# 4l3x4ndre/Metadata-Augmented-UNET-for-LST-NDVI

Measured on AMD Instinct MI355X. Metric: train images/sec (256x256x6->2 U-Net, B=32/GPU), higher is better.
Workload: dtype bf16; 1 GPU; metadata-unet base_filters=64, 32x6x256x256 tiles + 4-dim metadata per GPU, fwd+MSE+bwd+AdamW (src/train.py:243-256); global_batch=32, parallelism=dp1, sync_bn=False, launch=hipGraph replay of the captured step

## Files before the change

### include/mau_hip.h

```cpp
#ifndef MAU_HIP_H
#define MAU_HIP_H

#include <stddef.h>
#include <stdint.h>

#ifdef __cplusplus
extern "C" {
#endif

#define MAU_F32 0
#define MAU_BF16 1
#define MAU_F16 2

#define MAU_OK 0
#define MAU_ERR_ARG 1
#define MAU_ERR_HIP 2
#define MAU_ERR_DEVICE 3

typedef void* mau_stream_t;

#define MAU_ABI_VERSION 5
int mau_abi_version(void);
const char* mau_last_error(void);
int mau_device_check(void);

int mau_nchw_to_nhwc(const float* src, void* dst, int dtype, int N, int C, int H, int W, int ld,
                     mau_stream_t stream);
int mau_nhwc_to_nchw(const void* src, float* dst, int dtype, int N, int C, int H, int W, int ld,
                     mau_stream_t stream);

int mau_pack_tile_onehot(const unsigned char* cls_a, const unsigned char* cls_b, const float* cont,
                         const unsigned char* flip, void* out, int ldo, int dtype, int N, int H, int W,
                         int num_classes, int ncont, mau_stream_t stream);
int mau_flip_rows(const float* src, float* dst, const unsigned char* flip, int N, int C, int H, int W,
                  mau_stream_t stream);

int mau_conv3x3_kc(int dtype);
size_t mau_conv3x3_packed_elems(int dtype, int nout, int nin);
int mau_conv3x3_pack_weights(const float* w_oihw, void* wf, void* wd, int dtype, int Cout, int Cin,
                             mau_stream_t stream);
size_t mau_conv3x3_pack_desc_bytes(void);
int mau_conv3x3_pack_desc_fill(void* descs_host, int index, const float* w_oihw, void* wf, void* wd, int dtype, int Cout,
                               int Cin, int tile0, int* next_tile_host);
int mau_conv3x3_pack_weights_multi(const void* descs, int n, int total_tiles, int dtype, mau_stream_t stream);
int mau_conv3x3_num_pixel_tiles(int dtype, int N, int H, int W, int Cout);
int mau_conv3x3_fwd_pool(const void* x, int ldx, int C0, const void* wpk, const float* bias, const float* post_scale,
                         const float* post_shift, void* y, int ldy, int Cout, void* pooled, int ldpool, int dtype, int N, int H,
                         int W, mau_stream_t stream);
int mau_conv3x3_variant(int dtype, int N, int H, int W, int Cin, int Cout, int* tile_rows_host, int* waves_host, int* cout_block_host,
                        int* k_groups_host);
int mau_conv3x3_first_max_channels(void);
int mau_conv3x3_first_rows(int N, int H, int W);
size_t mau_conv3x3_first_wgrad_ws_elems(int N, int H, int W, int Cout);
int mau_conv3x3_first_wgrad(const void* x8, const void* dz, int lddz, float* dw_oihw, float* ws, int Cin, int Cout, int dtype, int N,
                            int H, int W, mau_stream_t stream);
int mau_conv3x3_first_fwd(const float* x_nchw, int Cin, const float* w_oihw, const float* bias, const float* post_scale,
                          const float* post_shift, void* y, int ldy, int Cout, float* slab, void* x8, int dtype, int N, int H,
                          int W, mau_stream_t stream);
int mau_conv3x3_fwd(const void* x, int ldx, int C0, const float* emb, void* emb_ws, int E, const void* wpk,
                    const float* bias, const float* post_scale, const float* post_shift, void* y, int ldy,
                    int Cout, float* slab, int dtype, int N, int H, int W, mau_stream_t stream);
int mau_conv3x3_fwd2(const void* x, int ldx, int C0, const void* x1, int ldx1, int C1, const float* emb, void* emb_ws,
                     int E, const void* wpk, const float* bias, const float* post_scale, const float* post_shift,
                     void* y, int ldy, int Cout, float* slab, int dtype, int N, int H, int W, mau_stream_t stream);
int mau_conv3x3_wgrad_splits(int dtype, int N, int H, int W, int Cout, int Cin);
size_t mau_conv3x3_wgrad_acc_elems(int dtype, int N, int H, int W, int Cout, int Cin);
int mau_conv3x3_wgrad(const void* x, int ldx, int C0, const float* emb, void* emb_ws, int E, const void* dy,
                      int lddy, int Cout, float* acc, int dtype, int N, int H, int W, mau_stream_t stream);
int mau_conv3x3_wgrad2(const void* x, int ldx, int C0, const void* x1, int ldx1, int C1, const float* emb, void* emb_ws,
                       int E, const void* dy, int lddy, int Cout, float* acc, int dtype, int N, int H, int W,
                       mau_stream_t stream);
int mau_conv3x3_unpack_wgrad(const float* acc, int nsplit, float* dw_oihw, int Cout, int Cin,
                             mau_stream_t stream);

size_t mau_reduce_rows_ws_elems(int rows, int M);
int mau_reduce_tickets_elems(void);
int mau_reduce_rows_f64(const float* slab, int rows, int M, int ldrow, double* sums, double* ws, unsigned* tickets,
                        mau_stream_t stream);
int mau_reduce_rows_f64_f32(const float* slab, int rows, int M, int ldrow, double* sums, float* sums32,
                            double* ws, unsigned* tickets, double append, mau_stream_t stream);
int mau_reduce_rows_f32(const float* slab, int rows, int M, int ldrow, float* out, double* ws, unsigned* tickets,
                        mau_stream_t stream);
int mau_bn_stats_sums_f64(const float* slab, int rows, int C, double* sums, double* ws, unsigned* tickets, double append,
                          mau_stream_t stream);
int mau_bn_finalize_train(const double* sums, double count, const float* gamma, const float* beta,
                          float* running_mean, float* running_var, int64_t* num_batches_tracked,
                          float momentum, float eps, float* scale, float* shift, float* mean,
                          float* invstd, int C, mau_stream_t stream);
size_t mau_bn_stats_ws_elems(int rows, int C);
int mau_bn_stats_finalize_train(const float* slab, int rows, double count, const float* gamma, const float* beta,
                                float* running_mean, float* running_var, int64_t* num_batches_tracked,
                                float momentum, float eps, float* scale, float* shift, float* mean, float* invstd,
                                double* ws, unsigned* tickets, int C, mau_stream_t stream);
int mau_bn_coeffs_eval(const float* gamma, const float* beta, const float* running_mean,
                       const float* running_var, float eps, float* scale, float* shift, float* mean,
                       float* invstd, int C, mau_stream_t stream);
int mau_bn_relu_apply(const void* y, int ldy, const float* scale, const float* shift, void* a, int lda,
                      int dtype, int64_t npix, int C, mau_stream_t stream);
int mau_bn_relu_apply_pool(const void* y, int ldy, const float* scale, const float* shift, void* a, int lda,
                           void* pooled, int ldp, unsigned short* argidx, int dtype, int N, int H, int W, int C,
                           mau_stream_t stream);
int mau_bn_relu_bwd_reduce(const void* da, int ldda, const void* y, int ldy, const float* scale,
                           const float* shift, const float* mean, const float* invstd, float* slab,
                           int ldslab, int dtype, int64_t npix, int C, mau_stream_t stream);
int mau_bn_relu_bwd_apply(const void* da, int ldda, const void* y, int ldy, const float* scale,
                          const float* shift, const float* mean, const float* invstd, const double* sums,
                          double count, void* dy, int lddy, int dtype, int64_t npix, int C,
                          mau_stream_t stream);
// ... 127 lines not shown
```

### metadata-augmented-unet-for-lst-ndvi_amd/_lib.py

```python
from __future__ import annotations

import ctypes as C
import os

import torch

_HERE = os.path.dirname(os.path.abspath(__file__))
LIB_PATH = os.environ.get("MAU_LIB") or os.path.join(_HERE, "libmau_hip.so")

MAU_F32 = 0
MAU_BF16 = 1
MAU_F16 = 2
MAU_OPT_ADAMW, MAU_OPT_ADAM, MAU_OPT_SGD = 0, 1, 2

_p, _i, _i64, _f, _d, _sz = C.c_void_p, C.c_int, C.c_int64, C.c_float, C.c_double, C.c_size_t

PROTOTYPES = {
    "mau_abi_version": (_i, []),
    "mau_last_error": (C.c_char_p, []),
    "mau_device_check": (_i, []),
    "mau_nchw_to_nhwc": (_i, [_p, _p, _i, _i, _i, _i, _i, _i, _p]),
    "mau_pack_tile_onehot": (_i, [_p, _p, _p, _p, _p, _i, _i, _i, _i, _i, _i, _i, _p]),
    "mau_flip_rows": (_i, [_p, _p, _p, _i, _i, _i, _i, _p]),
    "mau_nhwc_to_nchw": (_i, [_p, _p, _i, _i, _i, _i, _i, _i, _p]),
    "mau_conv3x3_kc": (_i, [_i]),
    "mau_conv3x3_packed_elems": (_sz, [_i, _i, _i]),
    "mau_conv3x3_pack_weights": (_i, [_p, _p, _p, _i, _i, _i, _p]),
    "mau_conv3x3_pack_desc_bytes": (_sz, []),
    "mau_conv3x3_pack_desc_fill": (_i, [_p, _i, _p, _p, _p, _i, _i, _i, _i, _p]),
    "mau_conv3x3_pack_weights_multi": (_i, [_p, _i, _i, _i, _p]),
    "mau_conv3x3_num_pixel_tiles": (_i, [_i, _i, _i, _i, _i]),
    "mau_conv3x3_variant": (_i, [_i, _i, _i, _i, _i, _i, _p, _p, _p, _p]),
    "mau_conv3x3_first_max_channels": (_i, []),
    "mau_conv3x3_first_rows": (_i, [_i, _i, _i]),
    "mau_conv3x3_first_wgrad_ws_elems": (_sz, [_i, _i, _i, _i]),
    "mau_conv3x3_first_wgrad": (_i, [_p, _p, _i, _p, _p, _i, _i, _i, _i, _i, _i, _p]),
    "mau_conv3x3_first_fwd": (_i, [_p, _i, _p, _p, _p, _p, _p, _i, _i, _p, _p, _i, _i, _i, _i, _p]),
    "mau_conv3x3_fwd": (_i, [_p, _i, _i, _p, _p, _i, _p, _p, _p, _p, _p, _i, _i, _p, _i, _i, _i, _i, _p]),
    "mau_conv3x3_fwd_pool": (_i, [_p, _i, _i, _p, _p, _p, _p, _p, _i, _i, _p, _i, _i, _i, _i, _i, _p]),
    "mau_conv3x3_fwd2": (_i, [_p, _i, _i, _p, _i, _i, _p, _p, _i, _p, _p, _p, _p, _p, _i, _i, _p, _i, _i, _i, _i, _p]),
    "mau_conv3x3_wgrad_splits": (_i, [_i, _i, _i, _i, _i, _i]),
    "mau_conv3x3_wgrad_acc_elems": (_sz, [_i, _i, _i, _i, _i, _i]),
    "mau_conv3x3_wgrad": (_i, [_p, _i, _i, _p, _p, _i, _p, _i, _i, _p, _i, _i, _i, _i, _p]),
    "mau_conv3x3_wgrad2": (_i, [_p, _i, _i, _p, _i, _i, _p, _p, _i, _p, _i, _i, _p, _i, _i, _i, _i, _p]),
    "mau_conv3x3_unpack_wgrad": (_i, [_p, _i, _p, _i, _i, _p]),
    "mau_reduce_rows_ws_elems": (_sz, [_i, _i]),
    "mau_reduce_tickets_elems": (_i, []),
    "mau_reduce_rows_f64": (_i, [_p, _i, _i, _i, _p, _p, _p, _p]),
    "mau_reduce_rows_f64_f32": (_i, [_p, _i, _i, _i, _p, _p, _p, _p, _d, _p]),
    "mau_reduce_rows_f32": (_i, [_p, _i, _i, _i, _p, _p, _p, _p]),
    "mau_bn_stats_sums_f64": (_i, [_p, _i, _i, _p, _p, _p, _d, _p]),
    "mau_bn_finalize_train": (_i, [_p, _d, _p, _p, _p, _p, _p, _f, _f, _p, _p, _p, _p, _i, _p]),
    "mau_bn_stats_ws_elems": (_sz, [_i, _i]),
    "mau_bn_stats_finalize_train": (_i, [_p, _i, _d, _p, _p, _p, _p, _p, _f, _f, _p, _p, _p, _p, _p, _p, _i, _p]),
    "mau_bn_coeffs_eval": (_i, [_p, _p, _p, _p, _f, _p, _p, _p, _p, _i, _p]),
    "mau_bn_relu_apply": (_i, [_p, _i, _p, _p, _p, _i, _i, _i64, _i, _p]),
    "mau_bn_relu_apply_pool": (_i, [_p, _i, _p, _p, _p, _i, _p, _i, _p, _i, _i, _i, _i, _i, _p]),
    "mau_bn_relu_bwd_reduce": (_i, [_p, _i, _p, _i, _p, _p, _p, _p, _p, _i, _i, _i64, _i, _p]),
    "mau_bn_relu_bwd_apply": (_i, [_p, _i, _p, _i, _p, _p, _p, _p, _p, _d, _p, _i, _i, _i64, _i, _p]),
    "mau_bn_bwd_rows": (_i, [_i64]),
    "mau_pool_bn_bwd_reduce": (_i, [_p, _i, _p, _i, _p, _p, _i, _p, _p, _p, _p, _p, _i, _i, _i, _i, _i, _i, _p]),
    "mau_pool_bn_bwd_apply": (_i, [_p, _i, _p, _i, _p, _p, _i, _p, _p, _p, _p, _p, _d, _p, _i, _i, _i, _i, _i, _i, _p]),
    "mau_head_bn_max_channels": (_i, []),
    "mau_head_bn_fwd": (_i, [_p, _i, _p, _p, _p, _p, _p, _i, _i, _i, _i, _i, _i, _p]),
    "mau_head_bn_bwd_reduce": (_i, [_p, _i, _p, _p, _p, _p, _p, _p, _p, _p, _i, _p, _i, _i, _i, _i, _i, _i, _p]),
    "mau_head_bn_bwd_apply": (_i, [_p, _i, _p, _p, _p, _p, _p, _d, _p, _p, _p, _p, _i, _i, _i, _i, _i, _i, _i, _p]),
    "mau_resize_bilinear_bn_fwd": (_i, [_p, _i, _i, _i, _p, _p, _p, _i, _i, _i, _i, _i, _i, _i, _p]),
    "mau_maxpool2x2_fwd": (_i, [_p, _i, _p, _i, _i, _i, _i, _i, _i, _p]),
    "mau_maxpool2x2_bwd": (_i, [_p, _i, _p, _i, _p, _i, _i, _i, _i, _i, _i, _p]),
    "mau_maxpool2x2_bwd_add": (_i, [_p, _i, _p, _i, _p, _i, _p, _i, _i, _i, _i, _i, _i, _p]),
    "mau_resize_bilinear_fwd": (_i, [_p, _i, _i, _i, _p, _i, _i, _i, _i, _i, _i, _i, _p]),
    "mau_resize_bilinear_bwd": (_i, [_p, _i, _i, _i, _i, _p, _i, _i, _i, _i, _i, _i, _p]),
    "mau_copy_channels": (_i, [_p, _i, _p, _i, _i, _i, _i, _i64, _i, _p]),
    "mau_bcast_fill": (_i, [_p, _p, _i, _i, _i, _i, _i, _i, _i, _p]),
    "mau_bcast_bwd_ws_elems": (_sz, [_i, _i, _i]),
    "mau_bcast_bwd": (_i, [_p, _i, _i, _p, _p, _i, _i, _i, _i, _p]),
    "mau_head_fwd": (_i, [_p, _i, _p, _p, _p, _i, _i, _i, _i, _i, _i, _p]),
    "mau_head_mean_ws_elems": (_sz, [_i, _i, _i]),
    "mau_head_mean": (_i, [_p, _i, _p, _p, _p, _p, _p, _p, _p, _i, _i, _i, _i, _i, _i, _p]),
    "mau_head_bwd": (_i, [_p, _i, _p, _p, _p, _p, _i, _p, _i, _i, _i, _i, _i, _i, _p]),
    "mau_head_bwd_rows": (_i, [_i, _i]),
    "mau_head_bwd_rowlen": (_i, [_i, _i]),
    "mau_meta_mlp_fwd": (_i, [_p, _p, _p, _p, _p, _p, _p, _i, _i, _i, _i, _p]),
    "mau_meta_mlp_bwd": (_i, [_p, _p, _p, _p, _p, _p, _p, _p, _p, _p, _i, _i, _i, _i, _p]),
    "mau_lstm_max_hidden": (_i, []),
    "mau_lstm_fwd": (_i, [_p, _p, _p, _p, _p, _p, _p, _p, _i, _i, _i, _p]),
    "mau_lstm_bwd_ws_elems": (_sz, [_i, _i, _i]),
    "mau_lstm_bwd": (_i, [_p, _p, _p, _p, _p, _p, _p, _p, _p, _p, _i, _i, _i, _p]),
    "mau_linear_fwd": (_i, [_p, _p, _p, _p, _i, _i, _i, _p]),
# ... 67 lines not shown
```

### metadata-augmented-unet-for-lst-ndvi_amd/csrc/conv3x3_first.hip

```cpp
#include "igemm_bf16_util.h"

namespace mau {
namespace first {
using namespace igemm;

constexpr int TH = 16, TW = 64, HR = TH + 2, HC = TW + 2, HPIX = HR * HC;
constexpr int NT = 256, NWAVE = NT / 64;
constexpr int LOADS = (HPIX + NT - 1) / NT;
typedef float f32x4v __attribute__((ext_vector_type(4)));

struct P {
  const float* x;
  int Cin;
  const float* w;
  const float* bias;
  const float* post_scale;
  const float* post_shift;
  void* y;
  int ldy, Cout, CoutPad;
  float* slab;
  void* x8;
  int N, H, W, tilesX, tilesY, nTiles;
};

// ... 264 lines not shown

int mau_conv3x3_first_rows(int N, int H, int W) {
  if (N <= 0 || H <= 0 || W <= 0) return 0;
  return mau::first::grid_x(N * mau::ceil_div(H, mau::first::TH) * mau::ceil_div(W, mau::first::TW));
}

int mau_conv3x3_first_fwd(const float* x, int Cin, const float* w, const float* bias, const float* post_scale, const float* post_shift, void* y,
                          int ldy, int Cout, float* slab, void* x8, int dtype, int N, int H, int W, mau_stream_t stream) {
  using namespace mau;
  MAU_REQUIRE(x && w && y && N > 0 && H > 0 && W > 0 && Cout > 0, "conv3x3_first_fwd: bad arguments");
  MAU_REQUIRE(Cin >= 1 && Cin <= 8, "conv3x3_first_fwd: %d input channels (this kernel serves <= 8; use mau_conv3x3_fwd)", Cin);
  MAU_REQUIRE(dtype == MAU_BF16 || dtype == MAU_F16, "conv3x3_first_fwd: 16-bit activation types only (fp32 = parity mode: mau_conv3x3_fwd)");
  MAU_REQUIRE(ldy % 8 == 0 && ldy >= Cout, "conv3x3_first_fwd: ldy must be a multiple of 8 and >= Cout");
  MAU_REQUIRE((post_scale == nullptr) == (post_shift == nullptr), "conv3x3_first_fwd: post_scale and post_shift come together");
  MAU_REQUIRE(!(post_scale != nullptr && slab != nullptr), "conv3x3_first_fwd: post_scale/post_shift and the statistics slab are mutually exclusive");
  MAU_REQUIRE((long long)N * H * W * ldy * 2 < (1ll << 40), "conv3x3_first_fwd: tensor too large");
  first::P p;
  p.x = x;
  p.Cin = Cin;
  p.w = w;
  p.bias = bias;
  p.post_scale = post_scale;
  p.post_shift = post_shift;
  p.y = y;
  p.ldy = ldy;
  p.Cout = Cout;
  p.CoutPad = round_up(Cout, 64);
  p.slab = slab;
  p.x8 = x8;
  p.N = N;
  p.H = H;
  p.W = W;
  p.tilesX = ceil_div(W, first::TW);
  p.tilesY = ceil_div(H, first::TH);
  p.nTiles = N * p.tilesX * p.tilesY;
  return dtype == MAU_F16 ? first::launch<true>(p, (hipStream_t)stream) : first::launch<false>(p, (hipStream_t)stream);
}

}

namespace mau {
namespace firstw {
using namespace igemm;
typedef float f32x4v __attribute__((ext_vector_type(4)));
typedef unsigned u32x2 __attribute__((ext_vector_type(2)));

constexpr int TWW = 32;
constexpr int DZ_BYTES = TWW * 128;
constexpr int XROW = 1024;
constexpr int BUF = DZ_BYTES + 3 * XROW;
constexpr int NT = 256, NWAVE = 4, NDMA = 7;
constexpr int NBT = 6, NCOL = 16 * NBT;

struct WP {
  const void* x8;
  const void* dz;
  int lddz, Cout;
  float* ws;
  int N, H, W, tilesX, nTiles;
};

template <bool F16>
__device__ __forceinline__ void mfma(const u32x4& a, const u32x4& b, f32x4v& c) {
  if constexpr (F16) asm volatile("v_mfma_f32_16x16x32_f16 %0, %1, %2, %0" : "+v"(c) : "v"(a), "v"(b));
  else asm volatile("v_mfma_f32_16x16x32_bf16 %0, %1, %2, %0" : "+v"(c) : "v"(a), "v"(b));
}
template <int OFF_HI>
__device__ __forceinline__ u32x4 tr_frag(unsigned addr_lo, unsigned addr_hi) {
  u32x2 lo, hi;
  asm volatile("ds_read_b64_tr_b16 %0, %2\n\tds_read_b64_tr_b16 %1, %3 offset:%4" : "=&v"(lo), "=&v"(hi) : "v"(addr_lo), "v"(addr_hi), "n"(OFF_HI));
  return __builtin_shufflevector(lo, hi, 0, 1, 2, 3);
}

template <bool F16>
__global__ __launch_bounds__(NT, 2) void first_wgrad_kernel(WP p) {
  extern __shared__ __attribute__((aligned(16))) unsigned char smem[];
  const int tid = threadIdx.x, lane = tid & 63;
  const int wave = __builtin_amdgcn_readfirstlane(tid >> 6);
  const int co0 = blockIdx.y * 64;
  const unsigned lds0 = (unsigned)(size_t)((__attribute__((address_space(3))) unsigned char*)smem) + wave * (2 * BUF);
  const unsigned long long dz_a = (unsigned long long)p.dz, x_a = (unsigned long long)p.x8, zero_a = (unsigned long long)g_zero_page;

  const int dz_px = lane >> 3, dz_ch = lane & 7;
  const bool dz_ch_ok = co0 + 8 * dz_ch < p.lddz;
  auto issue = [&](int tile, int buf) {
    const int txi = tile % p.tilesX, rowi = tile / p.tilesX;
    const int x0 = txi * TWW, y = rowi % p.H;
    unsigned char* dst = smem + wave * (2 * BUF) + buf * BUF;
#pragma unroll
    for (int d = 0; d < 4; ++d) {
      const int gx = x0 + 8 * d + dz_px;
      unsigned long long src = dz_a + 2ull * ((unsigned long long)((long long)rowi * p.W + gx) * (unsigned)p.lddz + (unsigned)(co0 + 8 * dz_ch));
      asm volatile("" : "+v"(src));
      src = (gx < p.W && dz_ch_ok) ? src : zero_a;
      __builtin_amdgcn_global_load_lds((glb_ptr)src, (lds_ptr)(dst + d * 1024), 16, 0, 0);
    }
#pragma unroll
    for (int dy = 0; dy < 3; ++dy) {
      const int gy = y + dy - 1, gx = x0 + lane - 1;
      const bool in = lane < TWW + 2 && gy >= 0 && gy < p.H && gx >= 0 && gx < p.W;
      unsigned long long src = x_a + 16ull * (unsigned long long)((long long)(rowi + dy - 1) * p.W + gx);
      asm volatile("" : "+v"(src));
      src = in ? src : zero_a;
      __builtin_amdgcn_global_load_lds((glb_ptr)src, (lds_ptr)(dst + DZ_BYTES + dy * XROW), 16, 0, 0);
    }
  };
  const int g = lane >> 4, q = (lane >> 2) & 3, pq = lane & 3;
  const unsigned a_lane = (unsigned)((8 * g + q) * 128 + 8 * pq);
  unsigned b_lane[NBT];
#pragma unroll
  for (int j = 0; j < NBT; ++j) b_lane[j] = (unsigned)(DZ_BYTES + (j >> 1) * XROW + (8 * g + q + 2 * (j & 1)) * 16 + 8 * pq);
  f32x4v acc[4][NBT];
#pragma unroll
  for (int t = 0; t < 4; ++t)
#pragma unroll
    for (int j = 0; j < NBT; ++j) acc[t][j] = f32x4v{0.f, 0.f, 0.f, 0.f};

  const int nw = gridDim.x * NWAVE, w0 = blockIdx.x * NWAVE + wave;
  int buf = 0;
  if (w0 < p.nTiles) issue(w0, 0);
  for (int tile = w0; tile < p.nTiles; tile += nw) {
    const bool more = tile + nw < p.nTiles;
    if (more) {
      issue(tile + nw, buf ^ 1);
      wait_vmcnt<NDMA>();
    } else {
      wait_vmcnt<0>();
    }
    const unsigned base = lds0 + buf * BUF;
    u32x4 A[4], B[NBT];
#pragma unroll
    for (int t = 0; t < 4; ++t) A[t] = tr_frag<4 * 128>(base + a_lane + 32 * t, base + a_lane + 32 * t);
#pragma unroll
    for (int j = 0; j < NBT; ++j) B[j] = tr_frag<4 * 16>(base + b_lane[j], base + b_lane[j]);
    asm volatile("s_waitcnt lgkmcnt(0)" ::: "memory");
#pragma unroll
    for (int t = 0; t < 4; ++t)
#pragma unroll
      for (int j = 0; j < NBT; ++j) mfma<F16>(A[t], B[j], acc[t][j]);
    buf ^= 1;
  }
  wait_vmcnt<0>();
  __syncthreads();
  float* red = reinterpret_cast<float*>(smem);
  const int dn = lane & 15, dq = lane >> 4;
  for (int wv = 0; wv < NWAVE; ++wv) {
    if (wave == wv) {
#pragma unroll
      for (int t = 0; t < 4; ++t)
#pragma unroll
        for (int j = 0; j < NBT; ++j)
#pragma unroll
          for (int r = 0; r < 4; ++r) {
            float* e = red + (16 * t + 4 * dq + r) * NCOL + 16 * j + dn;
            *e = wv == 0 ? acc[t][j][r] : *e + acc[t][j][r];
          }
    }
    __syncthreads();
  }
  float* out = p.ws + ((size_t)blockIdx.x * gridDim.y + blockIdx.y) * 64 * NCOL;
  for (int i = tid; i < 64 * NCOL; i += NT) out[i] = red[i];
}

constexpr int SUM_SL = 8, SUM_EL = 32;
__global__ __launch_bounds__(SUM_SL * SUM_EL) void first_wgrad_sum_kernel(const float* __restrict__ ws, int nwg, int coTiles, float* __restrict__ dw, int Cout, int Cin) {
  __shared__ float part[SUM_SL][SUM_EL];
  const int el = threadIdx.x % SUM_EL, sl = threadIdx.x / SUM_EL;
  const int i = blockIdx.x * SUM_EL + el, total = Cout * Cin * 9;
  const int ic = i < total ? i : 0;
  const int tap = ic % 9, ci = (ic / 9) % Cin, co = ic / (9 * Cin);
  const int dy = tap / 3, dx = tap - 3 * dy;
  const int col = 16 * (2 * dy + (dx == 2)) + 8 * (dx == 1) + ci;
  const float* src = ws + (size_t)co * NCOL + col;
  const size_t stride = (size_t)coTiles * 64 * NCOL;
  float s = 0.f;
  int wgi = sl;
  for (; wgi + 7 * SUM_SL < nwg; wgi += 8 * SUM_SL) {
    float v[8];
#pragma unroll
    for (int u = 0; u < 8; ++u) v[u] = src[(size_t)(wgi + u * SUM_SL) * stride];
#pragma unroll
    for (int u = 0; u < 8; ++u) s += v[u];
  }
  for (; wgi < nwg; wgi += SUM_SL) s += src[(size_t)wgi * stride];
  part[sl][el] = s;
  __syncthreads();
  if (sl == 0 && i < total) {
    float o = part[0][el];
#pragma unroll
    for (int k = 1; k < SUM_SL; ++k) o += part[k][el];
    dw[i] = o;
  }
}

static int grid_x(int nTiles) {
  const int cap = device_shape().cus * 2;
  const int need = ceil_div(nTiles, NWAVE);
  return need < cap ? need : cap;
}
}
}

extern "C" {

size_t mau_conv3x3_first_wgrad_ws_elems(int N, int H, int W, int Cout) {
  if (N <= 0 || H <= 0 || W <= 0 || Cout <= 0) return 0;
  return (size_t)mau::firstw::grid_x(N * H * mau::ceil_div(W, mau::firstw::TWW)) * mau::round_up(Cout, 64) * mau::firstw::NCOL;
}

int mau_conv3x3_first_wgrad(const void* x8, const void* dz, int lddz, float* dw, float* ws, int Cin, int Cout, int dtype, int N, int H, int W,
                            mau_stream_t stream) {
  using namespace mau;
  MAU_REQUIRE(x8 && dz && dw && ws && N > 0 && H > 0 && W > 0 && Cout > 0, "conv3x3_first_wgrad: bad arguments");
  MAU_REQUIRE(Cin >= 1 && Cin <= 8, "conv3x3_first_wgrad: %d input channels (this kernel serves <= 8; use mau_conv3x3_wgrad2)", Cin);
  MAU_REQUIRE(dtype == MAU_BF16 || dtype == MAU_F16, "conv3x3_first_wgrad: 16-bit activation types only");
  MAU_REQUIRE(lddz % 8 == 0 && lddz >= Cout && ((uintptr_t)x8 % 16) == 0 && ((uintptr_t)dz % 16) == 0, "conv3x3_first_wgrad: bad lddz / alignment");
  firstw::WP p;
  p.x8 = x8;
  p.dz = dz;
  p.lddz = lddz;
  p.Cout = Cout;
  p.ws = ws;
  p.N = N;
  p.H = H;
  p.W = W;
  p.tilesX = ceil_div(W, firstw::TWW);
  p.nTiles = N * H * p.tilesX;
  const int coTiles = round_up(Cout, 64) / 64;
  const dim3 grid(firstw::grid_x(p.nTiles), coTiles);
  constexpr size_t lds = (size_t)firstw::NWAVE * 2 * firstw::BUF;
  static_assert(lds >= 64 * firstw::NCOL * sizeof(float), "the cross-wave sum fits the DMA buffers");
  hipStream_t st = (hipStream_t)stream;
  if (dtype == MAU_F16) {
    MAU_LDS_ATTR(lds, &firstw::first_wgrad_kernel<true>);
    MAU_LAUNCH(firstw::first_wgrad_kernel<true>, grid, dim3(firstw::NT), lds, st, p);
  } else {
    MAU_LDS_ATTR(lds, &firstw::first_wgrad_kernel<false>);
    MAU_LAUNCH(firstw::first_wgrad_kernel<false>, grid, dim3(firstw::NT), lds, st, p);
  }
  const int rc = check_launch("first_wgrad_kernel");
  if (rc != MAU_OK) return rc;
  MAU_LAUNCH(firstw::first_wgrad_sum_kernel, dim3(ceil_div(Cout * Cin * 9, firstw::SUM_EL)), dim3(firstw::SUM_SL * firstw::SUM_EL), 0, st, ws, (int)grid.x,
             coTiles, dw, Cout, Cin);
  return check_launch("first_wgrad_sum_kernel");
}

}
```

### metadata-augmented-unet-for-lst-ndvi_amd/functional.py

```python
from __future__ import annotations

import contextlib
import dataclasses

import os
from dataclasses import dataclass
from typing import List, Optional, Sequence, Tuple

import torch

from . import _lib
from ._lib import MAU_BF16, MAU_F16, MAU_F32, call, lib

BN_EPS = 1e-5
BN_MOMENTUM = 0.1


def pad8(c: int) -> int:
    return (c + 7) // 8 * 8


def dtype_code(dt: torch.dtype) -> int:
    if dt == torch.float32:
        return MAU_F32
# ... 194 lines not shown
    @staticmethod
    def backward(ctx, g):
        g = _as_nhwc(g)
        N, H, W, _ = g.shape
        out = torch.empty((N, ctx.C, H, W), dtype=torch.float32, device=g.device)
        call("mau_nhwc_to_nchw", g.data_ptr(), out.data_ptr(), dtype_code(g.dtype), N, ctx.C, H, W, _ld(g), _stream())
        return out, None


def to_nchw(a: Act) -> torch.Tensor:
    t = _as_nhwc(a.t.detach())
    N, H, W, _ = t.shape
    out = torch.empty((N, a.C, H, W), dtype=torch.float32, device=t.device)
    call("mau_nhwc_to_nchw", t.data_ptr(), out.data_ptr(), dtype_code(t.dtype), N, a.C, H, W, _ld(t), _stream())
    return out


@dataclass
class BNState:
    training: bool
    C0: int
    momentum: float = BN_MOMENTUM
    eps: float = BN_EPS
    group: object = None
    comm: object = None
    world: int = 1
    grad_enabled: bool = True
    frozen: object = None
    C1: int = 0
    pool: bool = False
    out_view: object = None
    head: object = None
    up_to: object = None
    first: bool = False
    dtype: object = None
    dgrad_first: bool = False


def _all_reduce_(t: torch.Tensor, st: BNState):
    if st.comm is not None:
        st.comm.all_reduce(t, 0, _stream())
    elif st.group is not None:
        from .dist import all_reduce_sum
        all_reduce_sum(t, st.group)


_OVERLAP_WGRAD = int(os.environ.get("MAU_OVERLAP_WGRAD", "2") or 0)
_FUSED_REDUCE = True
_FUSED_BN = True
_FUSED_UP = True
_PACK_MULTI = True
_INFER_POOL_FUSED = True
_FIRST_WGRAD = True
_SIDE_STREAMS = {}


def _side_stream(dev) -> "torch.cuda.Stream":
    s = _SIDE_STREAMS.get(dev)
    if s is None:
        s = _SIDE_STREAMS[dev] = torch.cuda.Stream(device=dev)
    return s


def _join_side_when_backward_ends(dev):
    def join():
        torch.cuda.current_stream(dev).wait_stream(_side_stream(dev))

    torch.autograd.Variable._execution_engine.queue_callback(join)


_DGRAD_FIRST = None


def _conv_fwd(x, x1, st, emb, emb_ws, E, wpk, bias, post, y, Cout, slab, code, N, H, W, stream):
    scale, shift = post if post is not None else (None, None)
    call("mau_conv3x3_fwd2", x.data_ptr(), _ld(x), st.C0, x1.data_ptr() if x1 is not None else None,
         _ld(x1) if x1 is not None else 0, st.C1 if x1 is not None else 0, emb.data_ptr() if E else None,
         emb_ws.data_ptr() if E else None, E, wpk.data_ptr(), bias.data_ptr() if bias is not None else None,
         scale.data_ptr() if scale is not None else None, shift.data_ptr() if shift is not None else None,
         y.data_ptr(), _ld(y), Cout, slab.data_ptr() if slab is not None else None, code, N, H, W, stream)


class ConvBNReLU(torch.autograd.Function):

    @staticmethod
    def forward(ctx, x, x1, emb, weight, bias, gamma, beta, rmean, rvar, nbt, hw, hb, st: BNState):
        _require_cuda(x, "conv3x3")
        first = st.first
        if first:
            if x1 is not None or emb is not None or x.dim() != 4 or x.shape[1] != st.C0 or st.C0 > lib.mau_conv3x3_first_max_channels():
                raise RuntimeError("conv3x3 (first layer): expects one (N, C <= 8, H, W) fp32 input")
            xin = x.contiguous().float()
            N, _, H, W = xin.shape
            act_dt = st.dtype
        else:
            x = _as_nhwc(x)
            if x1 is not None:
                x1 = _as_nhwc(x1)
            N, H, W, _ = x.shape
            act_dt = x.dtype
        code = dtype_code(act_dt)
        dev = x.device
        Cout, Cin = weight.shape[0], weight.shape[1]
        E = 0 if emb is None else emb.shape[1]
        C1 = st.C1 if x1 is not None else 0
        if st.C0 + C1 + E != Cin:
# ... 133 lines not shown
            up = torch.empty((N, Hu, Wu, ldy), dtype=act_dt, device=dev)
            call("mau_resize_bilinear_bn_fwd", y.data_ptr(), ldy, H, W, scale.data_ptr(), shift.data_ptr(), up.data_ptr(), ldy, 0, code,
                 N, Hu, Wu, Cout, stream)
        else:
            a = dst if dst is not None else torch.empty_like(y)
            lda = _ld(a)
            if st.pool and H >= 2 and W >= 2:
                pl = torch.empty((N, H // 2, W // 2, ldy), dtype=act_dt, device=dev)
                argidx = torch.empty((N, H // 2, W // 2, ldy // 8), dtype=torch.int16, device=dev) if fused else None
                call("mau_bn_relu_apply_pool", y.data_ptr(), ldy, scale.data_ptr(), shift.data_ptr(), a.data_ptr(), lda,
                     pl.data_ptr(), ldy, argidx.data_ptr() if argidx is not None else None, code, N, H, W, Cout, stream)
            else:
                call("mau_bn_relu_apply", y.data_ptr(), ldy, scale.data_ptr(), shift.data_ptr(), a.data_ptr(), lda, code,
                     npix, Cout, stream)
            if st.head is not None:
                out = head_of(a)
            elif st.up_to is not None:
                up = up_of(a)
        ctx.st = st if st.out_view is None else dataclasses.replace(st, out_view=None)
        ctx.E = E
        ctx.C1 = C1
        ctx.wd = wd
        ctx.pooled = pl is not None
        ctx.head = (Co, tanh0, tuple(hw.shape), fuse_head) if st.head is not None else None
        ctx.up = (st.up_to, fuse_up) if st.up_to is not None else None
        keep_a = a if ((pl is not None and not fused) or (st.head is not None and not fuse_head)) else None
        ctx.save_for_backward(x, x1, emb, weight, y, scale, shift, mean, invstd, keep_a, w2, out, argidx)
        if st.head is not None:
            return out
        if st.up_to is not None:
            return up
        if st.pool:
            return a, pl
        return a

    @staticmethod
    def backward(ctx, da, dpl=None):
        x, x1, emb, weight, y, scale, shift, mean, invstd, a, w2, out, argidx = ctx.saved_tensors
        st: BNState = ctx.st
        E, C1 = ctx.E, ctx.C1
        N, H, W, ldy = y.shape
        code = dtype_code(y.dtype)
        dev = y.device
        Cout, Cin = weight.shape[0], weight.shape[1]
        npix = N * H * W
        stream = _stream()
        f32 = dict(dtype=torch.float32, device=dev)
        needs = ctx.needs_input_grad
        sync = st.training and st.group is not None
        rows = lib.mau_bn_bwd_rows(npix)
        slab = torch.empty((rows, 2 * Cout), **f32)
        sums = torch.empty(2 * Cout + 1, dtype=torch.float64, device=dev)
        g32 = torch.empty(2 * Cout, **f32)
        dy = torch.empty_like(y)
        dhw = dhb = None
        cptrs = (scale.data_ptr(), shift.data_ptr(), mean.data_ptr(), invstd.data_ptr())

        def finish_sums():
            ws = torch.empty(lib.mau_reduce_rows_ws_elems(rows, 2 * Cout), dtype=torch.float64, device=dev)
            call("mau_reduce_rows_f64_f32", slab.data_ptr(), rows, 2 * Cout, 2 * Cout, sums.data_ptr(), g32.data_ptr(), ws.data_ptr(),
                 _tickets(dev).data_ptr() if (_FUSED_REDUCE or sync) else None, float(npix) if sync else 0.0, stream)
            if not st.training:
                return torch.zeros_like(sums), float(npix)
            if sync:
                _all_reduce_(sums, st)
                return sums, 0.0
            return sums, float(npix)

        fused_pool = ctx.pooled and dpl is not None and argidx is not None
        if ctx.head is not None and ctx.head[3]:
            Co, tanh0, hshape, _ = ctx.head
            dout = da.contiguous().float()
            hrows, rowlen = lib.mau_head_bwd_rows(N, H * W), lib.mau_head_bwd_rowlen(Cout, Co)
            hslab = torch.empty((hrows, rowlen), **f32)
            call("mau_head_bn_bwd_reduce", y.data_ptr(), ldy, *cptrs, w2.data_ptr(), out.data_ptr(), dout.data_ptr(), slab.data_ptr(), Cout,
                 hslab.data_ptr(), tanh0, code, N, H * W, Cout, Co, stream)
            sums_apply, count = finish_sums()
            red = torch.empty(rowlen, **f32)
            hws = torch.empty(lib.mau_reduce_rows_ws_elems(hrows, rowlen), dtype=torch.float64, device=dev)
            call("mau_reduce_rows_f32", hslab.data_ptr(), hrows, rowlen, rowlen, red.data_ptr(), hws.data_ptr(),
                 _tickets(dev).data_ptr() if _FUSED_REDUCE else None, stream)
            red = red.view(Co, pad8(Cout) + 8)
            dhw = red[:, :Cout].reshape(hshape).contiguous()
            dhb = red[:, pad8(Cout)].contiguous()
            call("mau_head_bn_bwd_apply", y.data_ptr(), ldy, *cptrs, sums_apply.data_ptr(), count, w2.data_ptr(), out.data_ptr(),
                 dout.data_ptr(), dy.data_ptr(), ldy, tanh0, code, N, H * W, Cout, Co, stream)
        elif fused_pool:
            dpl = _as_nhwc(dpl)
            dsk = _as_nhwc(da) if da is not None else None
            pargs = (y.data_ptr(), ldy, dpl.data_ptr(), _ld(dpl), argidx.data_ptr(), dsk.data_ptr() if dsk is not None else None,
                     _ld(dsk) if dsk is not None else 0)
            call("mau_pool_bn_bwd_reduce", *pargs, *cptrs, slab.data_ptr(), Cout, code, N, H, W, Cout, stream)
            sums_apply, count = finish_sums()
            call("mau_pool_bn_bwd_apply", *pargs, *cptrs, sums_apply.data_ptr(), count, dy.data_ptr(), ldy, code, N, H, W, Cout, stream)
        else:
            if ctx.head is not None:
                Co, tanh0, hshape, _ = ctx.head
                dout = da.contiguous().float()
                da = torch.empty((N, H, W, ldy), dtype=y.dtype, device=dev)
                hrows, rowlen = lib.mau_head_bwd_rows(N, H * W), lib.mau_head_bwd_rowlen(Cout, Co)
                hslab = torch.empty((hrows, rowlen), **f32)
                call("mau_head_bwd", a.data_ptr(), _ld(a), w2.data_ptr(), out.data_ptr(), dout.data_ptr(), da.data_ptr(), ldy,
                     hslab.data_ptr(), tanh0, code, N, H * W, Cout, Co, stream)
                red = torch.empty(rowlen, **f32)
                hws = torch.empty(lib.mau_reduce_rows_ws_elems(hrows, rowlen), dtype=torch.float64, device=dev)
                call("mau_reduce_rows_f32", hslab.data_ptr(), hrows, rowlen, rowlen, red.data_ptr(), hws.data_ptr(),
                     _tickets(dev).data_ptr() if _FUSED_REDUCE else None, stream)
                red = red.view(Co, pad8(Cout) + 8)
                dhw = red[:, :Cout].reshape(hshape).contiguous()
                dhb = red[:, pad8(Cout)].contiguous()
            elif ctx.up is not None:
                (Hu, Wu), _ = ctx.up
                g = _as_nhwc(da)
                da = torch.empty((N, H, W, ldy), dtype=y.dtype, device=dev)
                call("mau_resize_bilinear_bwd", g.data_ptr(), _ld(g), 0, Hu, Wu, da.data_ptr(), ldy, code, N, H, W, Cout, stream)
            elif ctx.pooled and dpl is not None:
                dpl = _as_nhwc(dpl)
                act = a
                if act is None:
                    act = torch.empty_like(y)
                    call("mau_bn_relu_apply", y.data_ptr(), ldy, scale.data_ptr(), shift.data_ptr(), act.data_ptr(), ldy, code, npix, Cout, stream)
                dsum = torch.empty((N, H, W, ldy), dtype=y.dtype, device=dev)
                if da is None:
                    call("mau_maxpool2x2_bwd", act.data_ptr(), _ld(act), dpl.data_ptr(), _ld(dpl), dsum.data_ptr(), ldy, code, N, H, W, Cout, stream)
                else:
                    da = _as_nhwc(da)
                    call("mau_maxpool2x2_bwd_add", act.data_ptr(), _ld(act), dpl.data_ptr(), _ld(dpl), da.data_ptr(), _ld(da),
                         dsum.data_ptr(), ldy, code, N, H, W, Cout, stream)
                da = dsum
            elif da is None:
                da = torch.zeros((N, H, W, ldy), dtype=y.dtype, device=dev)
            da = _as_nhwc(da)
            call("mau_bn_relu_bwd_reduce", da.data_ptr(), _ld(da), y.data_ptr(), ldy, *cptrs, slab.data_ptr(), Cout, code, npix, Cout, stream)
            sums_apply, count = finish_sums()
            call("mau_bn_relu_bwd_apply", da.data_ptr(), _ld(da), y.data_ptr(), ldy, *cptrs, sums_apply.data_ptr(), count, dy.data_ptr(), ldy,
                 code, npix, Cout, stream)
        dgamma = g32[Cout:]
        dbeta = g32[:Cout]
        dw = None
        need_dx = needs[0] or (x1 is not None and needs[1]) or (E and needs[2])
        overlap = _OVERLAP_WGRAD
        side = _side_stream(dev) if (needs[3] and overlap and (need_dx or overlap >= 2)) else None
        deferred = False
        dfull = None
        if (st.dgrad_first if _DGRAD_FIRST is None else _DGRAD_FIRST == "1") and need_dx and needs[3] and side is not None:
            dy_ready = torch.cuda.Event()
            dy_ready.record()
            wd = ctx.wd if ctx.wd is not None else pack_conv_weights(weight, code, forward=False, dgrad=True)[1]
            dfull = torch.empty((N, H, W, pad8(Cin)), dtype=y.dtype, device=dev)
            call("mau_conv3x3_fwd", dy.data_ptr(), ldy, Cout, None, None, 0, wd.data_ptr(), None, None, None, dfull.data_ptr(),
                 pad8(Cin), Cin, None, code, N, H, W, stream)
            side.wait_event(dy_ready)
        if needs[3]:
            if side is not None and dfull is None:
                side.wait_stream(torch.cuda.current_stream())
            with torch.cuda.stream(side) if side is not None else contextlib.nullcontext():
                acc = torch.empty(max(lib.mau_conv3x3_wgrad_acc_elems(code, N, H, W, Cout, Cin),
                                      lib.mau_conv3x3_first_wgrad_ws_elems(N, H, W, Cout) if st.first else 0), **f32)
                emb_ws = torch.empty((N, E), dtype=y.dtype, device=dev) if E else None
            slot = getattr(weight, "_mau_grad_slot", None)
            dw = slot.view_as(weight) if (slot is not None and weight.is_leaf and weight.grad is None and slot.device == dev) else torch.empty_like(weight)
            wstream = side.cuda_stream if side is not None else stream
            deferred = side is not None and overlap >= 2 and weight.is_leaf and weight.grad is None
            if st.first and _FIRST_WGRAD:
                call("mau_conv3x3_first_wgrad", x.data_ptr(), dy.data_ptr(), ldy, dw.data_ptr(), acc.data_ptr(), Cin, Cout, code, N, H, W, wstream)
            else:
                call("mau_conv3x3_wgrad2", x.data_ptr(), _ld(x), st.C0, x1.data_ptr() if x1 is not None else None,
                     _ld(x1) if x1 is not None else 0, C1, emb.data_ptr() if E else None,
                     emb_ws.data_ptr() if E else None, E, dy.data_ptr(), ldy, Cout, acc.data_ptr(), code, N, H, W, wstream)
                call("mau_conv3x3_unpack_wgrad", acc.data_ptr(), lib.mau_conv3x3_wgrad_splits(code, N, H, W, Cout, Cin),
                     dw.data_ptr(), Cout, Cin, wstream)
            if deferred:
                for t in (x, x1, emb, dy, dw):
                    if t is not None:
                        t.record_stream(side)
                weight._mau_grad_stream = side
                _join_side_when_backward_ends(dev)
        dx = dx1 = demb = None
        if need_dx:
            wd = ctx.wd if ctx.wd is not None else pack_conv_weights(weight, code, forward=False, dgrad=True)[1]
            ldd = pad8(Cin)
            if dfull is None:
                dfull = torch.empty((N, H, W, ldd), dtype=y.dtype, device=dev)
                call("mau_conv3x3_fwd", dy.data_ptr(), ldy, Cout, None, None, 0, wd.data_ptr(), None, None, None, dfull.data_ptr(),
                     ldd, Cin, None, code, N, H, W, stream)
            Ct = st.C0 + C1
            if E and needs[2]:
                demb = torch.empty((N, E), **f32)
                ws = torch.empty(lib.mau_bcast_bwd_ws_elems(N, H * W, E), **f32)
                call("mau_bcast_bwd", dfull.data_ptr(), ldd, Ct, demb.data_ptr(), ws.data_ptr(), code, N, H * W, E, stream)
            if C1:
                if needs[0]:
                    dx = dfull[..., :st.C0]
                if needs[1]:
                    dx1 = dfull[..., st.C0:st.C0 + pad8(C1)]
            elif needs[0]:
                dx = dfull[..., :pad8(st.C0)] if E else dfull
        if side is not None and not deferred:
            torch.cuda.current_stream().wait_stream(side)
        dbias = None
        if needs[4]:
            if st.training:
                dbias = _zero_bias_grad(Cout, dev)
            else:
                dbias = scale * dbeta
        return dx, dx1, demb, dw, dbias, dgamma, dbeta, None, None, None, dhw, dhb, None


class MaxPool2x2(torch.autograd.Function):

    @staticmethod
    def forward(ctx, x, C):
        x = _as_nhwc(x)
        N, H, W, _ = x.shape
        ldy = pad8(C)
        y = torch.empty((N, H // 2, W // 2, ldy), dtype=x.dtype, device=x.device)
        call("mau_maxpool2x2_fwd", x.data_ptr(), _ld(x), y.data_ptr(), ldy, dtype_code(x.dtype), N, H, W, C, _stream())
        ctx.save_for_backward(x)
        ctx.C = C
        return y

    @staticmethod
    def backward(ctx, dy):
        (x,) = ctx.saved_tensors
        dy = _as_nhwc(dy)
        N, H, W, _ = x.shape
# ... 484 lines not shown
```

Baseline: 2563 images/s.

## Fuse BN-ReLU backward apply into first-layer weight-gradient kernel

For the first conv (input-only, no dx needed), the BatchNorm+ReLU backward apply is folded into the first-layer wgrad kernel. The kernel loads da and y directly, computes dz in registers, writes it to LDS and feeds the MFMA tiles. This removes the separate apply kernel and the full-resolution dy tensor write and read at 256x256x64. In exchange the wgrad kernel gets a new register-staged load pipeline with hand-counted vmcnt waits, more per-element ALU work, and extra streams to record for deferred execution.

```diff
diff --git a/include/mau_hip.h b/include/mau_hip.h
--- a/include/mau_hip.h
+++ b/include/mau_hip.h
@@ -54,6 +54,9 @@
 size_t mau_conv3x3_first_wgrad_ws_elems(int N, int H, int W, int Cout);
 int mau_conv3x3_first_wgrad(const void* x8, const void* dz, int lddz, float* dw_oihw, float* ws, int Cin, int Cout, int dtype, int N,
                             int H, int W, mau_stream_t stream);
+int mau_conv3x3_first_wgrad_bn(const void* x8, const void* da, int ldda, const void* y, int ldy, const float* scale, const float* shift,
+                               const float* mean, const float* invstd, const double* sums, double count, float* dw_oihw, float* ws,
+                               int Cin, int Cout, int dtype, int N, int H, int W, mau_stream_t stream);
 int mau_conv3x3_first_fwd(const float* x_nchw, int Cin, const float* w_oihw, const float* bias, const float* post_scale,
                           const float* post_shift, void* y, int ldy, int Cout, float* slab, void* x8, int dtype, int N, int H,
                           int W, mau_stream_t stream);
diff --git a/metadata-augmented-unet-for-lst-ndvi_amd/_lib.py b/metadata-augmented-unet-for-lst-ndvi_amd/_lib.py
--- a/metadata-augmented-unet-for-lst-ndvi_amd/_lib.py
+++ b/metadata-augmented-unet-for-lst-ndvi_amd/_lib.py
@@ -35,6 +35,7 @@
     "mau_conv3x3_first_rows": (_i, [_i, _i, _i]),
     "mau_conv3x3_first_wgrad_ws_elems": (_sz, [_i, _i, _i, _i]),
     "mau_conv3x3_first_wgrad": (_i, [_p, _p, _i, _p, _p, _i, _i, _i, _i, _i, _i, _p]),
+    "mau_conv3x3_first_wgrad_bn": (_i, [_p, _p, _i, _p, _i, _p, _p, _p, _p, _p, _d, _p, _p, _i, _i, _i, _i, _i, _i, _p]),
     "mau_conv3x3_first_fwd": (_i, [_p, _i, _p, _p, _p, _p, _p, _i, _i, _p, _p, _i, _i, _i, _i, _p]),
     "mau_conv3x3_fwd": (_i, [_p, _i, _i, _p, _p, _i, _p, _p, _p, _p, _p, _i, _i, _p, _i, _i, _i, _i, _p]),
     "mau_conv3x3_fwd_pool": (_i, [_p, _i, _i, _p, _p, _p, _p, _p, _i, _i, _p, _i, _i, _i, _i, _i, _p]),
diff --git a/metadata-augmented-unet-for-lst-ndvi_amd/csrc/conv3x3_first.hip b/metadata-augmented-unet-for-lst-ndvi_amd/csrc/conv3x3_first.hip
--- a/metadata-augmented-unet-for-lst-ndvi_amd/csrc/conv3x3_first.hip
+++ b/metadata-augmented-unet-for-lst-ndvi_amd/csrc/conv3x3_first.hip
@@ -340,13 +340,32 @@
 constexpr int NT = 256, NWAVE = 4, NDMA = 7;
 constexpr int NBT = 6, NCOL = 16 * NBT;
 
+constexpr int NLD = 8, NXDMA = 3;
+
 struct WP {
   const void* x8;
   const void* dz;
   int lddz, Cout;
   float* ws;
   int N, H, W, tilesX, nTiles;
+  const void* da;
+  int ldda;
+  const float *scale, *shift, *mean, *invstd;
+  const double* sums;
+  double inv_count;
 };
+
+struct Stage {
+  u32x4 g[4], v[4];
+  int xlim;
+};
+__device__ __forceinline__ void wait_stage(Stage& s) {
+  static_assert(NXDMA == 3, "the counted wait of the BN form");
+  asm volatile("s_waitcnt vmcnt(3)"
+               : "+v"(s.g[0]), "+v"(s.g[1]), "+v"(s.g[2]), "+v"(s.g[3]), "+v"(s.v[0]), "+v"(s.v[1]), "+v"(s.v[2]), "+v"(s.v[3])
+               :
+               : "memory");
+}
 
 template <bool F16>
 __device__ __forceinline__ void mfma(const u32x4& a, const u32x4& b, f32x4v& c) {
@@ -360,7 +379,7 @@
   return __builtin_shufflevector(lo, hi, 0, 1, 2, 3);
 }
 
-template <bool F16>
+template <bool F16, bool BN>
 __global__ __launch_bounds__(NT, 2) void first_wgrad_kernel(WP p) {
   extern __shared__ __attribute__((aligned(16))) unsigned char smem[];
   const int tid = threadIdx.x, lane = tid & 63;
@@ -405,16 +424,7 @@
     for (int j = 0; j < NBT; ++j) acc[t][j] = f32x4v{0.f, 0.f, 0.f, 0.f};
 
   const int nw = gridDim.x * NWAVE, w0 = blockIdx.x * NWAVE + wave;
-  int buf = 0;
-  if (w0 < p.nTiles) issue(w0, 0);
-  for (int tile = w0; tile < p.nTiles; tile += nw) {
-    const bool more = tile + nw < p.nTiles;
-    if (more) {
-      issue(tile + nw, buf ^ 1);
-      wait_vmcnt<NDMA>();
-    } else {
-      wait_vmcnt<0>();
-    }
+  auto multiply = [&](int buf) {
     const unsigned base = lds0 + buf * BUF;
     u32x4 A[4], B[NBT];
 #pragma unroll
@@ -426,7 +436,117 @@
     for (int t = 0; t < 4; ++t)
 #pragma unroll
       for (int j = 0; j < NBT; ++j) mfma<F16>(A[t], B[j], acc[t][j]);
-    buf ^= 1;
+  };
+  if constexpr (!BN) {
+    int buf = 0;
+    if (w0 < p.nTiles) issue(w0, 0);
+    for (int tile = w0; tile < p.nTiles; tile += nw) {
+      const bool more = tile + nw < p.nTiles;
+      if (more) {
+        issue(tile + nw, buf ^ 1);
+        wait_vmcnt<NDMA>();
+      } else {
+        wait_vmcnt<0>();
+      }
+      multiply(buf);
+      buf ^= 1;
+    }
+  } else {
+    using T = typename std::conditional<F16, f16, bf16>::type;
+    using T8 = typename std::conditional<F16, f16x8, bf16x8>::type;
+    const int C = p.Cout, c0 = co0 + 8 * dz_ch;
+    const bool ch_ok = c0 < ((C + 7) & ~7);
+    const unsigned long long da_a = (unsigned long long)p.da;
+    float sc[8], sh[8], k0[8], k1[8];
+    {
+      double inv_count = p.inv_count;
+      if (inv_count <= 0.0) inv_count = 1.0 / p.sums[2 * C];
+      double d1[8], d2[8];
+#pragma unroll
+      for (int j = 0; j < 8; ++j) {
+        sc[j] = coef(p.scale, c0 + j, C);
+        sh[j] = coef(p.shift, c0 + j, C);
+        k0[j] = coef(p.mean, c0 + j, C);
+        k1[j] = coef(p.invstd, c0 + j, C);
+        d1[j] = coef(p.sums, c0 + j, C);
+        d2[j] = coef(p.sums + C, c0 + j, C);
+      }
+#pragma unroll
+      for (int j = 0; j < 8; ++j) {
+        const float mu = k0[j], is = k1[j];
+        const float m1 = (float)(d1[j] * inv_count), m2 = (float)(d2[j] * inv_count);
+        k1[j] = __fmul_rn(__fmul_rn(sc[j], m2), is);
+        k0[j] = fmaf(sc[j], m1, -__fmul_rn(k1[j], mu));
+      }
+    }
+    asm volatile("s_waitcnt vmcnt(0)" ::: "memory");
+    auto load = [&](int tile, Stage& s) {
+      const bool tv = tile < p.nTiles;
+      const int tl = tv ? tile : 0;
+      const int txi = tl % p.tilesX, rowi = tl / p.tilesX, x0 = txi * TWW;
+      s.xlim = (tv && ch_ok) ? p.W - x0 - dz_px : 0;
+#pragma unroll
+      for (int d = 0; d < 4; ++d) {
+        const unsigned long long pix = (unsigned long long)((long long)rowi * p.W + (x0 + 8 * d + dz_px));
+        unsigned long long ga = da_a + 2ull * (pix * (unsigned)p.ldda + (unsigned)c0);
+        unsigned long long ya = dz_a + 2ull * (pix * (unsigned)p.lddz + (unsigned)c0);
+        asm volatile("" : "+v"(ga), "+v"(ya));
+        const bool ok = 8 * d < s.xlim;
+        ga = ok ? ga : da_a;
+        ya = ok ? ya : dz_a;
+        asm volatile("global_load_dwordx4 %0, %1, off" : "=v"(s.g[d]) : "v"(ga) : "memory");
+        asm volatile("global_load_dwordx4 %0, %1, off" : "=v"(s.v[d]) : "v"(ya) : "memory");
+      }
+    };
+    auto issue_x = [&](int tile, int buf) {
+      const bool tv = tile < p.nTiles;
+      const int tl = tv ? tile : 0;
+      const int txi = tl % p.tilesX, rowi = tl / p.tilesX;
+      const int x0 = txi * TWW, y = rowi % p.H;
+      unsigned char* dst = smem + wave * (2 * BUF) + buf * BUF;
+#pragma unroll
+      for (int dy = 0; dy < 3; ++dy) {
+        const int gy = y + dy - 1, gx = x0 + lane - 1;
+        const bool in = tv && lane < TWW + 2 && gy >= 0 && gy < p.H && gx >= 0 && gx < p.W;
+        unsigned long long src = x_a + 16ull * (unsigned long long)((long long)(rowi + dy - 1) * p.W + gx);
+        asm volatile("" : "+v"(src));
+        src = in ? src : zero_a;
+        __builtin_amdgcn_global_load_lds((glb_ptr)src, (lds_ptr)(dst + DZ_BYTES + dy * XROW), 16, 0, 0);
+      }
+    };
+    auto commit = [&](const Stage& s, int buf) {
+      const unsigned dst = lds0 + buf * BUF + lane * 16;
+#pragma unroll
+      for (int d = 0; d < 4; ++d) {
+        const T8 gv = __builtin_bit_cast(T8, s.g[d]), yv = __builtin_bit_cast(T8, s.v[d]);
+        T8 o;
+#pragma unroll
+        for (int j = 0; j < 8; ++j) {
+          const float g = F16 ? opaque((float)gv[j]) : (float)gv[j], y = F16 ? opaque((float)yv[j]) : (float)yv[j];
+          const float act = fmaf(y, sc[j], sh[j]);
+          const float dz = act > 0.f ? g : 0.f;
+          const float r = fmaf(sc[j], dz, -fmaf(k1[j], y, k0[j]));
+          o[j] = F16 ? (T)opaque(r) : (T)r;
+        }
+        u32x4 pk = __builtin_bit_cast(u32x4, o);
+        const bool ok = 8 * d < s.xlim;
+#pragma unroll
+        for (int i = 0; i < 4; ++i) pk[i] = ok ? pk[i] : 0u;
+        asm volatile("ds_write_b128 %0, %1 offset:%2" ::"v"(dst), "v"(pk), "n"(d * 1024) : "memory");
+      }
+    };
+    Stage s;
+    int buf = 0;
+    issue_x(w0, 0);
+    load(w0, s);
+    for (int tile = w0; tile < p.nTiles; tile += nw) {
+      issue_x(tile + nw, buf ^ 1);
+      wait_stage(s);
+      commit(s, buf);
+      load(tile + nw, s);
+      multiply(buf);
+      buf ^= 1;
+    }
   }
   wait_vmcnt<0>();
   __syncthreads();
@@ -496,6 +616,40 @@
   return (size_t)mau::firstw::grid_x(N * H * mau::ceil_div(W, mau::firstw::TWW)) * mau::round_up(Cout, 64) * mau::firstw::NCOL;
 }
 
+}
+
+namespace mau {
+namespace firstw {
+static int launch(WP& p, bool bn, float* dw, int Cin, int dtype, hipStream_t st) {
+  p.tilesX = ceil_div(p.W, TWW);
+  p.nTiles = p.N * p.H * p.tilesX;
+  const int coTiles = round_up(p.Cout, 64) / 64;
+  const dim3 grid(grid_x(p.nTiles), coTiles);
+  constexpr size_t lds = (size_t)NWAVE * 2 * BUF;
+  static_assert(lds >= 64 * NCOL * sizeof(float), "the cross-wave sum fits the DMA buffers");
+#define MAU_FIRSTW_LAUNCH(F16, BN)                                               \
+  do {                                                                           \
+    MAU_LDS_ATTR(lds, &first_wgrad_kernel<F16, BN>);                             \
+    MAU_LAUNCH((first_wgrad_kernel<F16, BN>), grid, dim3(NT), lds, st, p);       \
+  } while (0)
+  if (dtype == MAU_F16) {
+    if (bn) MAU_FIRSTW_LAUNCH(true, true);
+    else MAU_FIRSTW_LAUNCH(true, false);
+  } else {
+    if (bn) MAU_FIRSTW_LAUNCH(false, true);
+    else MAU_FIRSTW_LAUNCH(false, false);
+  }
+#undef MAU_FIRSTW_LAUNCH
+  const int rc = check_launch("first_wgrad_kernel");
+  if (rc != MAU_OK) return rc;
+  MAU_LAUNCH(first_wgrad_sum_kernel, dim3(ceil_div(p.Cout * Cin * 9, SUM_EL)), dim3(SUM_SL * SUM_EL), 0, st, p.ws, (int)grid.x, coTiles, dw, p.Cout, Cin);
+  return check_launch("first_wgrad_sum_kernel");
+}
+}
+}
+
+extern "C" {
+
 int mau_conv3x3_first_wgrad(const void* x8, const void* dz, int lddz, float* dw, float* ws, int Cin, int Cout, int dtype, int N, int H, int W,
                             mau_stream_t stream) {
   using namespace mau;
@@ -503,7 +657,7 @@
   MAU_REQUIRE(Cin >= 1 && Cin <= 8, "conv3x3_first_wgrad: %d input channels (this kernel serves <= 8; use mau_conv3x3_wgrad2)", Cin);
   MAU_REQUIRE(dtype == MAU_BF16 || dtype == MAU_F16, "conv3x3_first_wgrad: 16-bit activation types only");
   MAU_REQUIRE(lddz % 8 == 0 && lddz >= Cout && ((uintptr_t)x8 % 16) == 0 && ((uintptr_t)dz % 16) == 0, "conv3x3_first_wgrad: bad lddz / alignment");
-  firstw::WP p;
+  firstw::WP p = {};
   p.x8 = x8;
   p.dz = dz;
   p.lddz = lddz;
@@ -512,25 +666,39 @@
   p.N = N;
   p.H = H;
   p.W = W;
-  p.tilesX = ceil_div(W, firstw::TWW);
-  p.nTiles = N * H * p.tilesX;
-  const int coTiles = round_up(Cout, 64) / 64;
-  const dim3 grid(firstw::grid_x(p.nTiles), coTiles);
-  constexpr size_t lds = (size_t)firstw::NWAVE * 2 * firstw::BUF;
-  static_assert(lds >= 64 * firstw::NCOL * sizeof(float), "the cross-wave sum fits the DMA buffers");
-  hipStream_t st = (hipStream_t)stream;
-  if (dtype == MAU_F16) {
-    MAU_LDS_ATTR(lds, &firstw::first_wgrad_kernel<true>);
-    MAU_LAUNCH(firstw::first_wgrad_kernel<true>, grid, dim3(firstw::NT), lds, st, p);
-  } else {
-    MAU_LDS_ATTR(lds, &firstw::first_wgrad_kernel<false>);
-    MAU_LAUNCH(firstw::first_wgrad_kernel<false>, grid, dim3(firstw::NT), lds, st, p);
-  }
-  const int rc = check_launch("first_wgrad_kernel");
-  if (rc != MAU_OK) return rc;
-  MAU_LAUNCH(firstw::first_wgrad_sum_kernel, dim3(ceil_div(Cout * Cin * 9, firstw::SUM_EL)), dim3(firstw::SUM_SL * firstw::SUM_EL), 0, st, ws, (int)grid.x,
-             coTiles, dw, Cout, Cin);
-  return check_launch("first_wgrad_sum_kernel");
-}
-
-}
+  return firstw::launch(p, false, dw, Cin, dtype, (hipStream_t)stream);
+}
+
+int mau_conv3x3_first_wgrad_bn(const void* x8, const void* da, int ldda, const void* y, int ldy, const float* scale, const float* shift,
+                               const float* mean, const float* invstd, const double* sums, double count, float* dw, float* ws, int Cin,
+                               int Cout, int dtype, int N, int H, int W, mau_stream_t stream) {
+  using namespace mau;
+  MAU_REQUIRE(x8 && da && y && dw && ws && N > 0 && H > 0 && W > 0 && Cout > 0, "conv3x3_first_wgrad_bn: bad arguments");
+  MAU_REQUIRE(scale && shift && mean && invstd && sums && count >= 0, "conv3x3_first_wgrad_bn: bad BatchNorm arguments");
+  MAU_REQUIRE(Cin >= 1 && Cin <= 8, "conv3x3_first_wgrad_bn: %d input channels (this kernel serves <= 8)", Cin);
+  MAU_REQUIRE(dtype == MAU_BF16 || dtype == MAU_F16, "conv3x3_first_wgrad_bn: 16-bit activation types only");
+  const int C8 = round_up(Cout, 8);
+  MAU_REQUIRE(ldda % 8 == 0 && ldy % 8 == 0 && ldda >= C8 && ldy >= C8, "conv3x3_first_wgrad_bn: bad ldda / ldy");
+  MAU_REQUIRE(((uintptr_t)x8 % 16) == 0 && ((uintptr_t)da % 16) == 0 && ((uintptr_t)y % 16) == 0, "conv3x3_first_wgrad_bn: 16-byte alignment");
+  MAU_REQUIRE((long long)N * H * W * (ldda > ldy ? ldda : ldy) * 2 < (1ll << 40), "conv3x3_first_wgrad_bn: tensor too large");
+  firstw::WP p = {};
+  p.x8 = x8;
+  p.dz = y;
+  p.lddz = ldy;
+  p.Cout = Cout;
+  p.ws = ws;
+  p.N = N;
+  p.H = H;
+  p.W = W;
+  p.da = da;
+  p.ldda = ldda;
+  p.scale = scale;
+  p.shift = shift;
+  p.mean = mean;
+  p.invstd = invstd;
+  p.sums = sums;
+  p.inv_count = count > 0 ? 1.0 / count : 0.0;
+  return firstw::launch(p, true, dw, Cin, dtype, (hipStream_t)stream);
+}
+
+}
diff --git a/metadata-augmented-unet-for-lst-ndvi_amd/functional.py b/metadata-augmented-unet-for-lst-ndvi_amd/functional.py
--- a/metadata-augmented-unet-for-lst-ndvi_amd/functional.py
+++ b/metadata-augmented-unet-for-lst-ndvi_amd/functional.py
@@ -270,6 +270,7 @@
 _PACK_MULTI = True
 _INFER_POOL_FUSED = True
 _FIRST_WGRAD = True
+_FUSED_FIRST_BWD = True
 _SIDE_STREAMS = {}
 
 
@@ -509,7 +510,7 @@
         slab = torch.empty((rows, 2 * Cout), **f32)
         sums = torch.empty(2 * Cout + 1, dtype=torch.float64, device=dev)
         g32 = torch.empty(2 * Cout, **f32)
-        dy = torch.empty_like(y)
+        dy = None
         dhw = dhb = None
         cptrs = (scale.data_ptr(), shift.data_ptr(), mean.data_ptr(), invstd.data_ptr())
 
@@ -530,6 +531,7 @@
             dout = da.contiguous().float()
             hrows, rowlen = lib.mau_head_bwd_rows(N, H * W), lib.mau_head_bwd_rowlen(Cout, Co)
             hslab = torch.empty((hrows, rowlen), **f32)
+            dy = torch.empty_like(y)
             call("mau_head_bn_bwd_reduce", y.data_ptr(), ldy, *cptrs, w2.data_ptr(), out.data_ptr(), dout.data_ptr(), slab.data_ptr(), Cout,
                  hslab.data_ptr(), tanh0, code, N, H * W, Cout, Co, stream)
             sums_apply, count = finish_sums()
@@ -549,6 +551,7 @@
                      _ld(dsk) if dsk is not None else 0)
             call("mau_pool_bn_bwd_reduce", *pargs, *cptrs, slab.data_ptr(), Cout, code, N, H, W, Cout, stream)
             sums_apply, count = finish_sums()
+            dy = torch.empty_like(y)
             call("mau_pool_bn_bwd_apply", *pargs, *cptrs, sums_apply.data_ptr(), count, dy.data_ptr(), ldy, code, N, H, W, Cout, stream)
         else:
             if ctx.head is not None:
@@ -590,11 +593,16 @@
             da = _as_nhwc(da)
             call("mau_bn_relu_bwd_reduce", da.data_ptr(), _ld(da), y.data_ptr(), ldy, *cptrs, slab.data_ptr(), Cout, code, npix, Cout, stream)
             sums_apply, count = finish_sums()
-            call("mau_bn_relu_bwd_apply", da.data_ptr(), _ld(da), y.data_ptr(), ldy, *cptrs, sums_apply.data_ptr(), count, dy.data_ptr(), ldy,
-                 code, npix, Cout, stream)
+            fused_first = bool(st.first and _FIRST_WGRAD and _FUSED_FIRST_BWD and needs[3]
+                               and not (needs[0] or (x1 is not None and needs[1]) or (E and needs[2])))
+            if not fused_first:
+                dy = torch.empty_like(y)
+                call("mau_bn_relu_bwd_apply", da.data_ptr(), _ld(da), y.data_ptr(), ldy, *cptrs, sums_apply.data_ptr(), count, dy.data_ptr(), ldy,
+                     code, npix, Cout, stream)
         dgamma = g32[Cout:]
         dbeta = g32[:Cout]
         dw = None
+        fused_first = dy is None
         need_dx = needs[0] or (x1 is not None and needs[1]) or (E and needs[2])
         overlap = _OVERLAP_WGRAD
         side = _side_stream(dev) if (needs[3] and overlap and (need_dx or overlap >= 2)) else None
@@ -619,7 +627,10 @@
             dw = slot.view_as(weight) if (slot is not None and weight.is_leaf and weight.grad is None and slot.device == dev) else torch.empty_like(weight)
             wstream = side.cuda_stream if side is not None else stream
             deferred = side is not None and overlap >= 2 and weight.is_leaf and weight.grad is None
-            if st.first and _FIRST_WGRAD:
+            if fused_first:
+                call("mau_conv3x3_first_wgrad_bn", x.data_ptr(), da.data_ptr(), _ld(da), y.data_ptr(), ldy, *cptrs, sums_apply.data_ptr(), count,
+                     dw.data_ptr(), acc.data_ptr(), Cin, Cout, code, N, H, W, wstream)
+            elif st.first and _FIRST_WGRAD:
                 call("mau_conv3x3_first_wgrad", x.data_ptr(), dy.data_ptr(), ldy, dw.data_ptr(), acc.data_ptr(), Cin, Cout, code, N, H, W, wstream)
             else:
                 call("mau_conv3x3_wgrad2", x.data_ptr(), _ld(x), st.C0, x1.data_ptr() if x1 is not None else None,
@@ -628,7 +639,7 @@
                 call("mau_conv3x3_unpack_wgrad", acc.data_ptr(), lib.mau_conv3x3_wgrad_splits(code, N, H, W, Cout, Cin),
                      dw.data_ptr(), Cout, Cin, wstream)
             if deferred:
-                for t in (x, x1, emb, dy, dw):
+                for t in (x, x1, emb, dw) + ((da, y, scale, shift, mean, invstd, sums_apply) if fused_first else (dy,)):
                     if t is not None:
                         t.record_stream(side)
                 weight._mau_grad_stream = side
```

After: 2588 images/s (median of 6 runs). No clear change (+1.0%).
